# Hello1024/shared-tensor

Measured on AMD Instinct MI355X. Metric: async-DP tokens/sec GPT-2-small, higher is better.
Workload: dtype bf16; 1 GPU; model=gpt2-small, global_batch=64, seq_len=1024, parallelism=async-dp1, codec=1bit, n_params=124439808, paramsync=n/a at n_gpus=1 (no links)

## Files before the change

### build.py

```python
#!/usr/bin/env python3
import argparse
import hashlib
import os
import subprocess
import sysconfig

ROOT = os.path.dirname(os.path.abspath(__file__))
CSRC = os.path.join(ROOT, "sharedtensor_amd", "csrc")
OUT = os.path.join(ROOT, "sharedtensor_amd", "_core.so")
BUILD = os.path.join(ROOT, "build")

SOURCES = [
    "codec_cpu.cpp",
    "engine.cpp",
    "rccl_transport.cpp",
    "hip_kernels.hip",
    "ln_kernels.hip",
    "add_ln_kernels.hip",
    "add_rms_kernels.hip",
    "ce_kernels.hip",
    "gelu_kernels.hip",
    "swiglu_kernels.hip",
    "rope_kernels.hip",
    "bindings.cpp",
]

HEADERS = ["common.h", "codec_cpu.h", "engine.h", "hip_api.h", "rccl_transport.h"]


def pybind11_include():
    import pybind11
    return pybind11.get_include()


def build(force=False, debug=False, verbose=True):
    os.makedirs(BUILD, exist_ok=True)
    py_inc = sysconfig.get_paths()["include"]
    rocm = os.environ.get("ROCM_PATH", "/opt/rocm")
    hipcc = os.path.join(rocm, "bin", "hipcc")
    cxxflags = [
        "--offload-arch=gfx950",
        "-std=c++20",
        "-O3" if not debug else "-O0",
        "-g" if debug else "",
        "-fPIC",
        "-DSHAMD_WITH_HIP",
        f"-I{CSRC}",
        f"-I{py_inc}",
        f"-I{pybind11_include()}",
        f"-I{rocm}/include",
        "-Wno-unused-result",
        "-fvisibility=hidden",
        "-DNDEBUG" if not debug else "",
        "-parallel-jobs=4",
    ]
    cxxflags = [f for f in cxxflags if f]

    h = hashlib.sha256()
    for f in SOURCES + HEADERS:
        with open(os.path.join(CSRC, f), "rb") as fh:
            h.update(fh.read())
    h.update(" ".join(cxxflags).encode())
    stamp = os.path.join(BUILD, "core.stamp")
    digest = h.hexdigest()
    if not force and os.path.exists(OUT) and os.path.exists(stamp):
        with open(stamp) as fh:
            if fh.read().strip() == digest:
                if verbose:
                    print(f"[build.py] {OUT} up to date")
                return OUT

    objs = []
    procs = []
    for src in SOURCES:
        obj = os.path.join(BUILD, src.replace("/", "_") + ".o")
        objs.append(obj)
        cmd = [hipcc, "-c", os.path.join(CSRC, src), "-o", obj] + cxxflags
        if verbose:
            print("[build.py]", " ".join(cmd))
        procs.append(subprocess.Popen(cmd))
    rc = 0
    for p in procs:
        rc |= p.wait()
    if rc:
        raise RuntimeError("hipcc compilation failed")

    link = [hipcc, "-shared", "-fPIC", "-o", OUT] + objs + [
        f"-L{rocm}/lib", "-lamdhip64", "-lrccl", "-pthread",
        f"-Wl,-rpath,{rocm}/lib",
    ]
    if verbose:
        print("[build.py]", " ".join(link))
    subprocess.check_call(link)
    nm = subprocess.run(["nm", "-C", "-u", OUT], capture_output=True, text=True)
    bad = [l for l in nm.stdout.splitlines() if "shamd::" in l]
    if bad:
        raise RuntimeError("unresolved engine symbols:\n" + "\n".join(bad))
    with open(stamp, "w") as fh:
        fh.write(digest)
    if verbose:
        print(f"[build.py] built {OUT}")
    return OUT


if __name__ == "__main__":
    ap = argparse.ArgumentParser()
    ap.add_argument("--force", action="store_true")
    ap.add_argument("--debug", action="store_true")
    args = ap.parse_args()
    build(force=args.force, debug=args.debug)
```

### sharedtensor_amd/csrc/bindings.cpp

```cpp
#include <pybind11/pybind11.h>
#include <pybind11/stl.h>

#include <array>

#include "codec_cpu.h"
#include "engine.h"
#include "rccl_transport.h"

namespace py = pybind11;
using namespace shamd;

namespace {

py::tuple py_cpu_encode(int codec, uintptr_t delta, int64_t n, double scale_in,
                        uintptr_t payload_out) {
  Codec c = static_cast<Codec>(codec);
  float* d = reinterpret_cast<float*>(delta);
  float scale = scale_in < 0 ? cpu_compute_scale(c, d, n)
                             : static_cast<float>(scale_in);
  cpu_quantize(c, d, n, scale, reinterpret_cast<uint8_t*>(payload_out));
  return py::make_tuple(scale, payload_bytes(c, n));
}

void py_cpu_apply(int codec, uintptr_t payload, int64_t n, double scale,
// ... 133 lines not shown
                  reinterpret_cast<uint16_t*>(shadow_bf16),
                  static_cast<float>(lr), static_cast<float>(beta1),
                  static_cast<float>(beta2), static_cast<float>(eps),
                  static_cast<float>(wd), static_cast<float>(inv_bc1),
                  static_cast<float>(inv_bc2), n,
                  reinterpret_cast<float*>(d[0]),
                  reinterpret_cast<void*>(d[1]), reinterpret_cast<void*>(d[2]),
                  reinterpret_cast<void*>(d[3]), delta_bf16,
                  reinterpret_cast<hipStream_t>(stream));
}

void py_gpu_snapshot_capture(uintptr_t values, uintptr_t delta, uintptr_t out,
                             int64_t n, uintptr_t stream, bool delta_bf16) {
  hip_snapshot_capture(reinterpret_cast<const float*>(values),
                       reinterpret_cast<void*>(delta), delta_bf16,
                       reinterpret_cast<float*>(out), n,
                       reinterpret_cast<hipStream_t>(stream));
}

void py_gpu_add_delta_scatter(uintptr_t src, int64_t n,
                              std::vector<uintptr_t> dsts, uintptr_t stream,
                              bool delta_bf16) {
  uintptr_t d[3] = {0, 0, 0};
  for (size_t i = 0; i < dsts.size() && i < 3; ++i) d[i] = dsts[i];
  hip_add_delta_scatter(reinterpret_cast<const void*>(src), delta_bf16, n,
                        reinterpret_cast<float*>(d[0]),
                        reinterpret_cast<void*>(d[1]),
                        reinterpret_cast<void*>(d[2]),
                        reinterpret_cast<hipStream_t>(stream));
}

}

PYBIND11_MODULE(_core, m) {
  m.doc() = "MI355X-native shared-tensor engine (CDNA4 HIP + RCCL/TCP)";

  py::class_<Config>(m, "Config")
      .def(py::init<>())
      .def_readwrite("host", &Config::host)
      .def_readwrite("port", &Config::port)
      .def_readwrite("device", &Config::device)
      .def_property(
          "codec", [](const Config& c) { return static_cast<int>(c.codec); },
          [](Config& c, int v) { c.codec = static_cast<Codec>(v); })
      .def_readwrite("snapshot_join", &Config::snapshot_join)
      .def_readwrite("use_rccl", &Config::use_rccl)
      .def_readwrite("reconnect", &Config::reconnect)
      .def_readwrite("preserve_subtree", &Config::preserve_subtree)
      .def_readwrite("keepalive_s", &Config::keepalive_s)
      .def_readwrite("bw_limit", &Config::bw_limit)
      .def_readwrite("min_round_interval_s", &Config::min_round_interval_s)
      .def_readwrite("expected_children", &Config::expected_children)
      .def_readwrite("sizes", &Config::sizes)
      .def_readwrite("explicit_parent", &Config::explicit_parent)
      .def_readwrite("listen_port", &Config::listen_port)
      .def_readwrite("join_timeout_s", &Config::join_timeout_s)
      .def_readwrite("rms_sample_stride", &Config::rms_sample_stride)
      .def_readwrite("lagged_scale", &Config::lagged_scale)
      .def_readwrite("delta_bf16", &Config::delta_bf16)
      .def_readwrite("use_graphs", &Config::use_graphs);

  py::class_<Engine>(m, "Engine")
      .def(py::init<Config>())
      .def("set_values", &Engine::set_values)
      .def("set_link_buffers", &Engine::set_link_buffers)
      .def("start", &Engine::start, py::call_guard<py::gil_scoped_release>())
      .def("add_from", &Engine::add_from,
           py::call_guard<py::gil_scoped_release>())
      .def("copy_to", &Engine::copy_to,
           py::call_guard<py::gil_scoped_release>())
      .def("fused_sgd", &Engine::fused_sgd,
           py::call_guard<py::gil_scoped_release>())
      .def("fused_sgd_bf16", &Engine::fused_sgd_bf16,
           py::call_guard<py::gil_scoped_release>())
      .def("fused_adamw", &Engine::fused_adamw,
           py::call_guard<py::gil_scoped_release>())
      .def("notify_dirty", &Engine::notify_dirty)
      .def("close", &Engine::close, py::call_guard<py::gil_scoped_release>())
      .def("is_master", &Engine::is_master)
      .def("listen_port", &Engine::listen_port)
      .def("last_error", &Engine::last_error)
      .def("reconnect_count", &Engine::reconnect_count)
      .def("recent_scales_sent", &Engine::recent_scales_sent)
      .def("recent_scales_recv", &Engine::recent_scales_recv)
      .def("link_stats", [](Engine& e) {
        py::list out;
        for (auto& s : e.link_stats()) {
          py::dict d;
          d["rounds_sent"] = s.rounds_sent;
          d["rounds_recv"] = s.rounds_recv;
          d["bytes_sent"] = s.bytes_sent;
          d["bytes_recv"] = s.bytes_recv;
          d["last_scale_sent"] = s.last_scale_sent;
          d["last_scale_recv"] = s.last_scale_recv;
          d["active"] = s.active;
          d["dead"] = s.dead;
          d["peer"] = s.peer;
          d["rccl"] = s.rccl;
          out.append(d);
        }
        return out;
      });

  py::class_<DevCodec>(m, "DevCodec")
      .def(py::init<int, std::vector<int64_t>, int, bool>(), py::arg("codec"),
           py::arg("sizes"), py::arg("device"), py::arg("delta_bf16") = false)
      .def("reduce_scales", &DevCodec::reduce_scales)
      .def("quantize", &DevCodec::quantize, py::arg("delta"),
           py::arg("scales"), py::arg("payload"), py::arg("stream"),
           py::arg("stats") = 0)
      .def("finalize_scales", &DevCodec::finalize_scales)
      .def("apply", &DevCodec::apply);
  m.def("gpu_add_scatter", &py_gpu_add_scatter, py::arg("src"), py::arg("n"),
        py::arg("alpha"), py::arg("dsts"), py::arg("stream"),
        py::arg("delta_bf16") = false);
  m.def("gpu_fused_sgd", &py_gpu_fused_sgd, py::arg("mom"), py::arg("grad"),
        py::arg("lr"), py::arg("mu"), py::arg("n"), py::arg("dsts"),
        py::arg("stream"), py::arg("delta_bf16") = false);
  m.def("gpu_fused_sgd_bf16", &py_gpu_fused_sgd_bf16, py::arg("mom"),
        py::arg("grad"), py::arg("shadow"), py::arg("lr"), py::arg("mu"),
        py::arg("n"), py::arg("dsts"), py::arg("stream"),
        py::arg("delta_bf16") = false);
  m.def("gpu_fused_adamw", &py_gpu_fused_adamw, py::arg("mom"),
        py::arg("vel"), py::arg("grad"), py::arg("grad_bf16"),
        py::arg("shadow"), py::arg("lr"), py::arg("beta1"), py::arg("beta2"),
        py::arg("eps"), py::arg("wd"), py::arg("inv_bc1"), py::arg("inv_bc2"),
        py::arg("n"), py::arg("dsts"), py::arg("stream"),
        py::arg("delta_bf16") = false);
  m.def("gpu_snapshot_capture", &py_gpu_snapshot_capture, py::arg("values"),
        py::arg("delta"), py::arg("out"), py::arg("n"), py::arg("stream"),
        py::arg("delta_bf16") = false);
  m.def("gpu_add_delta_scatter", &py_gpu_add_delta_scatter, py::arg("src"),
        py::arg("n"), py::arg("dsts"), py::arg("stream"),
        py::arg("delta_bf16") = false);
  m.def("rccl_loopback_payload", &rccl_loopback_payload,
        "Self ncclSend/ncclRecv of a real payload on one device (1-rank "
        "comm): executes the non-blocking enqueue ordering + stream polling "
        "the 2-GPU xGMI links use and verifies the moved bytes.");
  m.def("rccl_self_test", &rccl_self_test,
        py::call_guard<py::gil_scoped_release>());

  m.def("gelu_fwd", [](uintptr_t x, uintptr_t y, int64_t n, uintptr_t stream) {
    hip_gelu_fwd(reinterpret_cast<const void*>(x), reinterpret_cast<void*>(y),
                 n, reinterpret_cast<hipStream_t>(stream));
  });
  m.def("gelu_bwd", [](uintptr_t dy, uintptr_t x, uintptr_t dx, int64_t n,
                       uintptr_t stream) {
    hip_gelu_bwd(reinterpret_cast<const void*>(dy),
                 reinterpret_cast<const void*>(x),
                 reinterpret_cast<void*>(dx), n,
                 reinterpret_cast<hipStream_t>(stream));
  });

  m.def("ce_fwd", [](uintptr_t logits, uintptr_t targets, uintptr_t loss,
                     uintptr_t row_m, uintptr_t row_lse, int64_t R, int64_t V,
                     uintptr_t stream) {
    hip_ce_fwd(reinterpret_cast<const void*>(logits),
               reinterpret_cast<const int32_t*>(targets),
               reinterpret_cast<float*>(loss), reinterpret_cast<float*>(row_m),
               reinterpret_cast<float*>(row_lse), R, V,
               reinterpret_cast<hipStream_t>(stream));
  });
  m.def("ce_bwd", [](uintptr_t logits, uintptr_t targets, uintptr_t row_lse,
                     uintptr_t dlogits, uintptr_t gscale_dev, double inv_r,
                     int64_t R, int64_t V, uintptr_t stream,
                     bool skip_if_unit) {
    hip_ce_bwd(reinterpret_cast<const void*>(logits),
               reinterpret_cast<const int32_t*>(targets),
               reinterpret_cast<const float*>(row_lse),
               reinterpret_cast<void*>(dlogits),
               reinterpret_cast<const float*>(gscale_dev),
               static_cast<float>(inv_r), R, V, skip_if_unit,
               reinterpret_cast<hipStream_t>(stream));
  }, py::arg("logits"), py::arg("targets"), py::arg("row_lse"),
     py::arg("dlogits"), py::arg("gscale_dev"), py::arg("inv_r"),
     py::arg("R"), py::arg("V"), py::arg("stream"),
     py::arg("skip_if_unit") = false);
  m.def("ce_fwd_grad", [](uintptr_t logits, uintptr_t targets, uintptr_t loss,
                          uintptr_t row_lse, uintptr_t dlogits, double inv_r,
                          int64_t R, int64_t V, uintptr_t stream) {
    hip_ce_fwd_grad(reinterpret_cast<const void*>(logits),
                    reinterpret_cast<const int32_t*>(targets),
                    reinterpret_cast<float*>(loss),
                    reinterpret_cast<float*>(row_lse),
                    reinterpret_cast<void*>(dlogits),
                    static_cast<float>(inv_r), R, V,
                    reinterpret_cast<hipStream_t>(stream));
  });
  m.def("ce_fwd_grad_max_v", &hip_ce_fwd_grad_max_v);

  m.def("ln_fwd", [](uintptr_t x, uintptr_t w, uintptr_t b, uintptr_t y,
                     uintptr_t mean, uintptr_t rstd, int64_t R, int C,
                     double eps, uintptr_t stream) {
    hip_ln_fwd(reinterpret_cast<const void*>(x),
               reinterpret_cast<const void*>(w),
               reinterpret_cast<const void*>(b), reinterpret_cast<void*>(y),
               reinterpret_cast<float*>(mean), reinterpret_cast<float*>(rstd),
               R, C, static_cast<float>(eps),
               reinterpret_cast<hipStream_t>(stream));
  });
  m.def("colsum_bf16", [](uintptr_t x, uintptr_t out, int64_t R, int C,
                          uintptr_t stream) {
    hip_colsum_bf16(reinterpret_cast<const void*>(x),
                    reinterpret_cast<float*>(out), R, C,
                    reinterpret_cast<hipStream_t>(stream));
  });
  m.def("swiglu_fwd", [](uintptr_t x1, uintptr_t x3, uintptr_t y, int64_t n,
                         uintptr_t stream) {
    hip_swiglu_fwd(reinterpret_cast<const void*>(x1),
                   reinterpret_cast<const void*>(x3),
                   reinterpret_cast<void*>(y), n,
                   reinterpret_cast<hipStream_t>(stream));
  });
  m.def("swiglu_bwd", [](uintptr_t dy, uintptr_t x1, uintptr_t x3,
                         uintptr_t dx1, uintptr_t dx3, int64_t n,
                         uintptr_t stream) {
    hip_swiglu_bwd(reinterpret_cast<const void*>(dy),
                   reinterpret_cast<const void*>(x1),
                   reinterpret_cast<const void*>(x3),
                   reinterpret_cast<void*>(dx1),
                   reinterpret_cast<void*>(dx3), n,
                   reinterpret_cast<hipStream_t>(stream));
  });
  m.def("rope_qk", [](uintptr_t q, uintptr_t k, uintptr_t q_out,
                      uintptr_t k_out, uintptr_t cos, uintptr_t sin,
                      int64_t B, int64_t Hq, int64_t Hkv, int64_t T,
                      int64_t D, std::array<int64_t, 3> q_strides,
                      std::array<int64_t, 3> k_strides,
                      std::array<int64_t, 3> q_out_strides,
                      std::array<int64_t, 3> k_out_strides, bool inverse,
                      uintptr_t stream) {
    auto st = [](const std::array<int64_t, 3>& a) {
      return RopeStrides{a[0], a[1], a[2]};
    };
    hip_rope_qk(reinterpret_cast<const void*>(q),
                reinterpret_cast<const void*>(k),
                reinterpret_cast<void*>(q_out),
                reinterpret_cast<void*>(k_out),
                reinterpret_cast<const float*>(cos),
                reinterpret_cast<const float*>(sin), B, Hq, Hkv, T, D,
                st(q_strides), st(k_strides), st(q_out_strides),
                st(k_out_strides), inverse,
                reinterpret_cast<hipStream_t>(stream));
  }, py::arg("q"), py::arg("k"), py::arg("q_out"), py::arg("k_out"),
     py::arg("cos"), py::arg("sin"), py::arg("B"), py::arg("Hq"),
     py::arg("Hkv"), py::arg("T"), py::arg("D"), py::arg("q_strides"),
     py::arg("k_strides"), py::arg("q_out_strides"),
     py::arg("k_out_strides"), py::arg("inverse"), py::arg("stream"));
  m.def("rms_fwd", [](uintptr_t x, uintptr_t w, uintptr_t y, uintptr_t rstd,
                      int64_t R, int C, double eps, uintptr_t stream) {
    hip_rms_fwd(reinterpret_cast<const void*>(x),
                reinterpret_cast<const void*>(w), reinterpret_cast<void*>(y),
                reinterpret_cast<float*>(rstd), R, C, static_cast<float>(eps),
                reinterpret_cast<hipStream_t>(stream));
  });
  m.def("rms_bwd", [](uintptr_t dy, uintptr_t x, uintptr_t w, uintptr_t rstd,
                      uintptr_t dx, uintptr_t dgamma, int64_t R, int C,
                      uintptr_t stream) {
    hip_rms_bwd(reinterpret_cast<const void*>(dy),
                reinterpret_cast<const void*>(x),
                reinterpret_cast<const void*>(w),
                reinterpret_cast<const float*>(rstd),
                reinterpret_cast<void*>(dx), reinterpret_cast<float*>(dgamma),
                R, C, reinterpret_cast<hipStream_t>(stream));
  });
  m.def("ln_bwd", [](uintptr_t dy, uintptr_t x, uintptr_t w, uintptr_t mean,
                     uintptr_t rstd, uintptr_t dx, uintptr_t dgamma,
                     uintptr_t dbeta, int64_t R, int C, uintptr_t stream) {
    hip_ln_bwd(reinterpret_cast<const void*>(dy),
               reinterpret_cast<const void*>(x),
               reinterpret_cast<const void*>(w),
               reinterpret_cast<const float*>(mean),
               reinterpret_cast<const float*>(rstd),
               reinterpret_cast<void*>(dx), reinterpret_cast<float*>(dgamma),
               reinterpret_cast<float*>(dbeta), R, C,
               reinterpret_cast<hipStream_t>(stream));
  });

  m.def("add_ln_supported", &hip_add_ln_supported);
  m.def("add_ln_max_blocks", &hip_add_ln_max_blocks);
  m.def("add_ln_fwd", [](uintptr_t x, uintptr_t delta, uintptr_t dbias,
                         uintptr_t w, uintptr_t b, uintptr_t x_new,
                         uintptr_t y, uintptr_t mean, uintptr_t rstd,
                         int64_t R, int C, double eps, uintptr_t stream) {
    hip_add_ln_fwd(reinterpret_cast<const void*>(x),
                   reinterpret_cast<const void*>(delta),
                   reinterpret_cast<const void*>(dbias),
                   reinterpret_cast<const void*>(w),
                   reinterpret_cast<const void*>(b),
                   reinterpret_cast<void*>(x_new), reinterpret_cast<void*>(y),
                   reinterpret_cast<float*>(mean),
                   reinterpret_cast<float*>(rstd), R, C,
                   static_cast<float>(eps),
                   reinterpret_cast<hipStream_t>(stream));
  });
  m.def("add_ln_bwd", [](uintptr_t dy, uintptr_t x_new, uintptr_t w,
                         uintptr_t mean, uintptr_t rstd, uintptr_t d_x_new,
                         uintptr_t dx_total, uintptr_t dgamma, uintptr_t dbeta,
                         uintptr_t ddbias, uintptr_t partial, int64_t R, int C,
                         uintptr_t stream) {
    hip_add_ln_bwd(reinterpret_cast<const void*>(dy),
                   reinterpret_cast<const void*>(x_new),
                   reinterpret_cast<const void*>(w),
                   reinterpret_cast<const float*>(mean),
                   reinterpret_cast<const float*>(rstd),
                   reinterpret_cast<const void*>(d_x_new),
// ... 56 lines not shown
```

### sharedtensor_amd/csrc/gelu_kernels.hip

```cpp
#include <hip/hip_runtime.h>

#include <stdexcept>
#include <string>

#include "hip_api.h"

namespace shamd {

#define HIP_CHECK_GL(expr)                                                 \
  do {                                                                     \
    hipError_t _e = (expr);                                                \
    if (_e != hipSuccess)                                                  \
      throw std::runtime_error(std::string("HIP error: ") +                \
                               hipGetErrorString(_e));                     \
  } while (0)

static __device__ __forceinline__ float gl_lo(uint32_t p) {
  return __uint_as_float(p << 16);
}
static __device__ __forceinline__ float gl_hi(uint32_t p) {
  return __uint_as_float(p & 0xFFFF0000u);
}
static __device__ __forceinline__ uint16_t gl_bf16(float f) {
  uint32_t u = __float_as_uint(f);
  if ((u & 0x7FFFFFFFu) > 0x7F800000u) return 0x7FC0;
  u += 0x7FFFu + ((u >> 16) & 1u);
  return static_cast<uint16_t>(u >> 16);
}
static __device__ __forceinline__ uint32_t gl_pack(float lo, float hi) {
  return static_cast<uint32_t>(gl_bf16(lo)) |
         (static_cast<uint32_t>(gl_bf16(hi)) << 16);
}

constexpr float GK = 0.7978845608028654f;
constexpr float GC = 0.044715f;

static __device__ __forceinline__ float gelu_f(float x) {
  float inner = GK * (x + GC * x * x * x);
  return 0.5f * x * (1.f + tanhf(inner));
}

static __device__ __forceinline__ float gelu_grad_f(float xin) {
  float x = fminf(fmaxf(xin, -10.f), 10.f);
  if (xin != xin) x = xin;
  float x2 = x * x;
  float inner = GK * x * (1.f + GC * x2);
  float t = tanhf(inner);
  float sech2 = 1.f - t * t;
  return 0.5f * (1.f + t) + 0.5f * x * sech2 * GK * (1.f + 3.f * GC * x2);
}

__global__ void k_gelu_fwd(const uint4* __restrict__ x,
                           uint4* __restrict__ y, int64_t n8) {
  int64_t g = static_cast<int64_t>(gridDim.x) * blockDim.x;
  for (int64_t i = blockIdx.x * (int64_t)blockDim.x + threadIdx.x; i < n8; i += g) {
    uint4 u = x[i];
    uint4 o;
    const uint32_t* up = &u.x;
    uint32_t* op = &o.x;
#pragma unroll
    for (int k = 0; k < 4; ++k)
      op[k] = gl_pack(gelu_f(gl_lo(up[k])), gelu_f(gl_hi(up[k])));
    y[i] = o;
  }
}

__global__ void k_gelu_bwd(const uint4* __restrict__ dy,
                           const uint4* __restrict__ x,
                           uint4* __restrict__ dx, int64_t n8) {
  int64_t g = static_cast<int64_t>(gridDim.x) * blockDim.x;
  for (int64_t i = blockIdx.x * (int64_t)blockDim.x + threadIdx.x; i < n8; i += g) {
    uint4 u = x[i], d = dy[i];
    uint4 o;
    const uint32_t* up = &u.x;
    const uint32_t* dp = &d.x;
    uint32_t* op = &o.x;
#pragma unroll
    for (int k = 0; k < 4; ++k)
      op[k] = gl_pack(gl_lo(dp[k]) * gelu_grad_f(gl_lo(up[k])),
                      gl_hi(dp[k]) * gelu_grad_f(gl_hi(up[k])));
    dx[i] = o;
  }
}

static void gelu_check_align(const void* p, const char* what) {
  if (reinterpret_cast<uintptr_t>(p) & 15u)
    throw std::runtime_error(std::string("gelu: ") + what +
                             " is not 16-byte aligned");
}

static inline int gelu_grid(int64_t npairs) {
  int64_t g = (npairs + 255) / 256;
  return static_cast<int>(g < 16384 ? (g > 0 ? g : 1) : 16384);
}

void hip_gelu_fwd(const void* x, void* y, int64_t n, hipStream_t s) {
  if (n % 8) throw std::runtime_error("gelu: n must be a multiple of 8");
  gelu_check_align(x, "x");
  gelu_check_align(y, "y");
  if (n <= 0) return;
  hipLaunchKernelGGL(k_gelu_fwd, dim3(gelu_grid(n / 8)), dim3(256), 0, s,
                     static_cast<const uint4*>(x),
                     static_cast<uint4*>(y), n / 8);
  HIP_CHECK_GL(hipGetLastError());
}

void hip_gelu_bwd(const void* dy, const void* x, void* dx, int64_t n,
                  hipStream_t s) {
  if (n % 8) throw std::runtime_error("gelu: n must be a multiple of 8");
  gelu_check_align(dy, "dy");
  gelu_check_align(x, "x");
  gelu_check_align(dx, "dx");
  if (n <= 0) return;
  hipLaunchKernelGGL(k_gelu_bwd, dim3(gelu_grid(n / 8)), dim3(256), 0, s,
                     static_cast<const uint4*>(dy),
                     static_cast<const uint4*>(x),
                     static_cast<uint4*>(dx), n / 8);
  HIP_CHECK_GL(hipGetLastError());
}

}
```

### sharedtensor_amd/csrc/hip_api.h

```cpp
#pragma once

#include <hip/hip_runtime.h>

#include "common.h"

namespace shamd {

inline int64_t align8(int64_t x) { return (x + 7) & ~int64_t(7); }

struct DevTable {
  int64_t* offs = nullptr;
  int64_t* poffs = nullptr;
  int T = 0;
  int64_t n = 0;
  int64_t pe = 0;
};


void hip_reduce_scales(Codec c, const void* delta, bool delta_bf16,
                       const DevTable& tb, void* reduce_buf, float* scales_out,
                       int sample_stride, hipStream_t s);

void hip_quantize(Codec c, void* delta, bool delta_bf16, const DevTable& tb,
                  const float* scales_dev, uint8_t* payload, hipStream_t s,
                  void* stats_out = nullptr);

void hip_finalize_scales(Codec c, const DevTable& tb, const void* reduce_buf,
                         float* scales_out, int sample_stride, hipStream_t s);

void hip_apply(Codec c, const uint8_t* payload, const DevTable& tb,
               const float* scales_dev, float* values, void* d1, void* d2,
               bool delta_bf16, hipStream_t s);

void hip_add_scatter(const float* src, int64_t n, float alpha, float* values,
                     void* d1, void* d2, void* d3, bool delta_bf16,
                     hipStream_t s);

void hip_snapshot_capture(const float* values, void* delta, bool delta_bf16,
                          float* out, int64_t n, hipStream_t s);

void hip_add_delta_scatter(const void* src_delta, bool delta_bf16, int64_t n,
                           float* values, void* d1, void* d2, hipStream_t s);

void hip_fused_sgd(float* mom, const float* grad, float lr, float momentum,
                   int64_t n, float* values, void* d1, void* d2, void* d3,
                   bool delta_bf16, hipStream_t s);

void hip_fused_sgd_bf16(float* mom, const uint16_t* grad, uint16_t* shadow,
                        float lr, float momentum, int64_t n, float* values,
                        void* d1, void* d2, void* d3, bool delta_bf16,
                        hipStream_t s);

void hip_fused_adamw(float* mom, float* vel, const void* grad, bool grad_bf16,
                     uint16_t* shadow, float lr, float beta1, float beta2,
                     float eps, float wd, float inv_bc1, float inv_bc2,
                     int64_t n, float* values, void* d1, void* d2, void* d3,
                     bool delta_bf16, hipStream_t s);

void hip_ln_fwd(const void* x, const void* w, const void* b, void* y,
                float* mean, float* rstd, int64_t R, int C, float eps,
                hipStream_t s);
void hip_ln_bwd(const void* dy, const void* x, const void* w,
                const float* mean, const float* rstd, void* dx, float* dgamma,
                float* dbeta, int64_t R, int C, hipStream_t s);

bool hip_add_ln_supported(int C);
int hip_add_ln_max_blocks();
void hip_add_ln_fwd(const void* x, const void* delta, const void* dbias,
                    const void* w, const void* b, void* x_new, void* y,
                    float* mean, float* rstd, int64_t R, int C, float eps,
                    hipStream_t s);
void hip_add_ln_bwd(const void* dy, const void* x_new, const void* w,
                    const float* mean, const float* rstd, const void* d_x_new,
                    void* dx_total, void* dgamma, void* dbeta, void* ddbias,
                    float* partial, int64_t R, int C, hipStream_t s);

void hip_colsum_bf16(const void* x, float* out, int64_t R, int C,
                     hipStream_t s);

void hip_rms_fwd(const void* x, const void* w, void* y, float* rstd,
                 int64_t R, int C, float eps, hipStream_t s);
void hip_rms_bwd(const void* dy, const void* x, const void* w,
                 const float* rstd, void* dx, float* dgamma, int64_t R, int C,
                 hipStream_t s);

bool hip_add_rms_supported(int C);
int hip_add_rms_max_blocks();
void hip_add_rms_fwd(const void* x, const void* delta, const void* w,
                     void* x_new, void* y, float* rstd, int64_t R, int C,
                     float eps, hipStream_t s);
void hip_add_rms_bwd(const void* dy, const void* x_new, const void* w,
                     const float* rstd, const void* d_x_new, void* dx_total,
                     void* dgamma, float* partial, int64_t R, int C,
                     hipStream_t s);

void hip_ce_fwd(const void* logits, const int32_t* targets, float* loss,
                float* row_m, float* row_lse, int64_t R, int64_t V,
                hipStream_t s);
void hip_ce_bwd(const void* logits, const int32_t* targets,
                const float* row_lse, void* dlogits, const float* gscale_dev,
                float inv_r, int64_t R, int64_t V, bool skip_if_unit,
                hipStream_t s);
int64_t hip_ce_fwd_grad_max_v();
void hip_ce_fwd_grad(const void* logits, const int32_t* targets, float* loss,
                     float* row_lse, void* dlogits, float inv_r, int64_t R,
                     int64_t V, hipStream_t s);

void hip_swiglu_fwd(const void* x1, const void* x3, void* y, int64_t n,
                    hipStream_t s);
void hip_swiglu_bwd(const void* dy, const void* x1, const void* x3, void* dx1,
                    void* dx3, int64_t n, hipStream_t s);

struct RopeStrides {
  int64_t b = 0, h = 0, t = 0;
};
void hip_rope_qk(const void* q, const void* k, void* q_out, void* k_out,
                 const float* cos, const float* sin, int64_t B, int64_t Hq,
                 int64_t Hkv, int64_t T, int64_t D, const RopeStrides& q_in,
                 const RopeStrides& k_in, const RopeStrides& q_os,
                 const RopeStrides& k_os, bool inverse, hipStream_t s);

void hip_gelu_fwd(const void* x, void* y, int64_t n, hipStream_t s);
void hip_gelu_bwd(const void* dy, const void* x, void* dx, int64_t n,
                  hipStream_t s);

}
```

### sharedtensor_amd/models/gpt2.py

```python
from __future__ import annotations

import math
from dataclasses import dataclass

import torch
import torch.nn as nn
import torch.nn.functional as F


@dataclass
class GPT2Config:
    vocab_size: int = 50257
    n_layer: int = 12
    n_head: int = 12
    n_embd: int = 768
    block_size: int = 1024
    dropout: float = 0.0

    @classmethod
    def small(cls):
        return cls()

    @classmethod
    def tiny(cls):
        return cls(vocab_size=256, n_layer=2, n_head=2, n_embd=64,
                   block_size=64)


FUSE_PROJ_BIAS = True


class FusedLayerNorm(nn.LayerNorm):

    def forward(self, x):
        if (x.is_cuda and x.dtype == torch.bfloat16
                and self.weight.dtype == torch.bfloat16):
            from ..ops import fused_ln
            if fused_ln.can_use(x, self.weight):
                return fused_ln.fused_layer_norm(x, self.weight, self.bias,
                                                 self.eps)
            with torch.autocast("cuda", enabled=False):
                return F.layer_norm(x, self.normalized_shape, self.weight,
                                    self.bias, self.eps)
        return super().forward(x)


def _fused_ln_ok(ln: nn.LayerNorm, x: torch.Tensor) -> bool:
    if (x.is_cuda and x.dtype == torch.bfloat16
            and ln.weight.dtype == torch.bfloat16):
        from ..ops import fused_ln
        return fused_ln.can_use(x, ln.weight)
    return False


def add_ln(ln: nn.LayerNorm, x, delta, delta_bias=None):
    if delta is None:
        return x, ln(x)
    if _fused_ln_ok(ln, x):
        from ..ops import fused_ln
        return fused_ln.fused_add_layer_norm(x, delta, ln.weight, ln.bias,
                                             ln.eps, delta_bias)
    x = x + delta
    if delta_bias is not None:
        x = x + delta_bias
    return x, ln(x)


class CausalSelfAttention(nn.Module):
    def __init__(self, cfg: GPT2Config):
        super().__init__()
        assert cfg.n_embd % cfg.n_head == 0
        self.qkv = nn.Linear(cfg.n_embd, 3 * cfg.n_embd)
        self.proj = nn.Linear(cfg.n_embd, cfg.n_embd)
        self.n_head = cfg.n_head
        self.head_dim = cfg.n_embd // cfg.n_head

    def forward(self, x, proj_bias=True):
        B, T, C = x.shape
        q, k, v = self.qkv(x).split(C, dim=2)
        q = q.view(B, T, self.n_head, self.head_dim).transpose(1, 2)
        k = k.view(B, T, self.n_head, self.head_dim).transpose(1, 2)
        v = v.view(B, T, self.n_head, self.head_dim).transpose(1, 2)
        if x.is_cuda:
            from torch.nn.attention import SDPBackend, sdpa_kernel
            with sdpa_kernel([SDPBackend.EFFICIENT_ATTENTION,
                              SDPBackend.FLASH_ATTENTION, SDPBackend.MATH],
                             set_priority=True):
                y = F.scaled_dot_product_attention(q, k, v, is_causal=True)
        else:
            y = F.scaled_dot_product_attention(q, k, v, is_causal=True)
        y = y.transpose(1, 2).contiguous().view(B, T, C)
        if not proj_bias:
            return F.linear(y, self.proj.weight)
        return self.proj(y)


class MLP(nn.Module):
    def __init__(self, cfg: GPT2Config):
        super().__init__()
        self.fc = nn.Linear(cfg.n_embd, 4 * cfg.n_embd)
        self.proj = nn.Linear(4 * cfg.n_embd, cfg.n_embd)

    def forward(self, x, proj_bias=True):
        h = F.gelu(self.fc(x), approximate="tanh")
        if not proj_bias:
            return F.linear(h, self.proj.weight)
        return self.proj(h)


class Block(nn.Module):
    def __init__(self, cfg: GPT2Config):
        super().__init__()
        self.ln1 = FusedLayerNorm(cfg.n_embd)
        self.attn = CausalSelfAttention(cfg)
        self.ln2 = FusedLayerNorm(cfg.n_embd)
        self.mlp = MLP(cfg)

    def forward(self, x, delta=None, delta_bias=None, fuse_proj_bias=False):
        x, h = add_ln(self.ln1, x, delta, delta_bias)
        fuse = fuse_proj_bias and _fused_ln_ok(self.ln2, x)
        a = self.attn(h, proj_bias=not fuse)
        x, h = add_ln(self.ln2, x, a, self.attn.proj.bias if fuse else None)
        m = self.mlp(h, proj_bias=not fuse)
        return x, m, (self.mlp.proj.bias if fuse else None)


class GPT2(nn.Module):
    def __init__(self, cfg: GPT2Config):
        super().__init__()
        self.cfg = cfg
        self.wte = nn.Embedding(cfg.vocab_size, cfg.n_embd)
        self.wpe = nn.Embedding(cfg.block_size, cfg.n_embd)
        self.blocks = nn.ModuleList(Block(cfg) for _ in range(cfg.n_layer))
        self.ln_f = FusedLayerNorm(cfg.n_embd)
        self.lm_head = nn.Linear(cfg.n_embd, cfg.vocab_size, bias=False)
        self.lm_head.weight = self.wte.weight
        self.apply(self._init)
        for name, p in self.named_parameters():
            if name.endswith("proj.weight"):
                nn.init.normal_(p, std=0.02 / math.sqrt(2 * cfg.n_layer))

    @staticmethod
    def _init(m):
        if isinstance(m, nn.Linear):
            nn.init.normal_(m.weight, std=0.02)
            if m.bias is not None:
                nn.init.zeros_(m.bias)
        elif isinstance(m, nn.Embedding):
            nn.init.normal_(m.weight, std=0.02)

    def forward(self, idx, targets=None):
        B, T = idx.shape
        pos = torch.arange(T, device=idx.device)
        x = self.wte(idx) + self.wpe(pos)
        delta = delta_bias = None
        for blk in self.blocks:
            x, delta, delta_bias = blk(x, delta, delta_bias,
                                       FUSE_PROJ_BIAS)
        _, x = add_ln(self.ln_f, x, delta, delta_bias)
        logits = self.lm_head(x)
        if targets is None:
            return logits, None
        flat = logits.view(-1, logits.size(-1))
        tgt = targets.reshape(-1)
        if flat.is_cuda and flat.dtype == torch.bfloat16:
            from ..ops import fused_ce
            if fused_ce.can_use(flat):
                return logits, fused_ce.fused_cross_entropy(flat, tgt)
        loss = F.cross_entropy(flat, tgt)
        return logits, loss

    def num_params(self) -> int:
        return sum(p.numel() for p in self.parameters())
```

Baseline: 783,500 tokens/s.

## Fuse QKV bias-grad column sum into split backward packing kernel

```diff
diff --git a/build.py b/build.py
--- a/build.py
+++ b/build.py
@@ -20,12 +20,13 @@
     "add_rms_kernels.hip",
     "ce_kernels.hip",
     "gelu_kernels.hip",
+    "bias_grad_kernels.hip",
     "swiglu_kernels.hip",
     "rope_kernels.hip",
     "bindings.cpp",
 ]
 
-HEADERS = ["common.h", "codec_cpu.h", "engine.h", "hip_api.h", "rccl_transport.h"]
+HEADERS = ["common.h", "codec_cpu.h", "engine.h", "gelu_math.h", "hip_api.h", "rccl_transport.h"]
 
 
 def pybind11_include():
diff --git a/sharedtensor_amd/csrc/bias_grad_kernels.hip b/sharedtensor_amd/csrc/bias_grad_kernels.hip
--- /dev/null
+++ b/sharedtensor_amd/csrc/bias_grad_kernels.hip
@@ -0,0 +1,242 @@
+#include <hip/hip_runtime.h>
+
+#include <stdexcept>
+#include <string>
+
+#include "gelu_math.h"
+#include "hip_api.h"
+
+namespace shamd {
+
+#define HIP_CHECK_BG(expr)                                                 \
+  do {                                                                     \
+    hipError_t _e = (expr);                                                \
+    if (_e != hipSuccess)                                                  \
+      throw std::runtime_error(std::string("HIP error: ") +                \
+                               hipGetErrorString(_e));                     \
+  } while (0)
+
+constexpr int BG_THREADS = 1024;
+constexpr int BG_TARGET_BLOCKS = 512;
+constexpr int BG_MAX_CT = 128;
+constexpr int BG_GELU_ROWS = 1;
+constexpr int BG_PACK_ROWS = 2;
+
+struct BgGeom {
+  int ct_shift;
+  int gx, gy;
+};
+
+static BgGeom bg_geom(int64_t R, int64_t n8, int rows) {
+  int shift = 0;
+  while ((2 << shift) <= BG_MAX_CT && n8 % (2 << shift) == 0) ++shift;
+  if (shift < 4) {
+    shift = 0;
+    while (shift < 4 && (1 << shift) < n8) ++shift;
+  }
+  BgGeom g;
+  g.ct_shift = shift;
+  const int ct = 1 << shift, rt = BG_THREADS >> shift;
+  const int64_t gx = (n8 + ct - 1) / ct;
+  if (gx > 65535) throw std::runtime_error("bias_grad: too many columns");
+  g.gx = static_cast<int>(gx);
+  int gymax = BG_TARGET_BLOCKS / g.gx;
+  if (gymax < 1) gymax = 1;
+  const int64_t need = (R + rows * rt - 1) / (rows * rt);
+  g.gy = static_cast<int>(need < gymax ? (need > 0 ? need : 1) : gymax);
+  return g;
+}
+
+static __device__ __forceinline__ void bg_acc(float* a, const uint4& o) {
+  const uint32_t* op = &o.x;
+#pragma unroll
+  for (int k = 0; k < 4; ++k) {
+    a[2 * k] += gl_lo(op[k]);
+    a[2 * k + 1] += gl_hi(op[k]);
+  }
+}
+
+static __device__ __forceinline__ void bg_block_partial(
+    const float* a, float* red, float* __restrict__ partial, int ct_shift,
+    int64_t N) {
+  float4* r4 = reinterpret_cast<float4*>(red);
+  r4[2 * threadIdx.x] = make_float4(a[0], a[1], a[2], a[3]);
+  r4[2 * threadIdx.x + 1] = make_float4(a[4], a[5], a[6], a[7]);
+  __syncthreads();
+  const int w = 8 << ct_shift;
+  const int rt = BG_THREADS >> ct_shift;
+  const int j = threadIdx.x;
+  const int64_t col = static_cast<int64_t>(blockIdx.x) * w + j;
+  if (j < w && col < N) {
+    float t = 0.f;
+    for (int y = 0; y < rt; ++y) t += red[y * w + j];
+    partial[static_cast<int64_t>(blockIdx.y) * N + col] = t;
+  }
+}
+
+static __device__ __forceinline__ uint4 bg_gelu_bwd8(const uint4& d,
+                                                     const uint4& u) {
+  uint4 o;
+  const uint32_t* up = &u.x;
+  const uint32_t* dp = &d.x;
+  uint32_t* op = &o.x;
+#pragma unroll
+  for (int k = 0; k < 4; ++k)
+    op[k] = gl_pack(gl_lo(dp[k]) * gelu_grad_f(gl_lo(up[k])),
+                    gl_hi(dp[k]) * gelu_grad_f(gl_hi(up[k])));
+  return o;
+}
+
+__global__ __launch_bounds__(BG_THREADS) void k_gelu_bwd_colsum(
+    const uint4* __restrict__ dy, const uint4* __restrict__ x,
+    uint4* __restrict__ dx, float* __restrict__ partial, int64_t R,
+    int64_t n8, int ct_shift) {
+  __shared__ float red[BG_THREADS * 8];
+  const int cx = threadIdx.x & ((1 << ct_shift) - 1);
+  const int ty = threadIdx.x >> ct_shift;
+  const int rt = BG_THREADS >> ct_shift;
+  const int64_t cj = (static_cast<int64_t>(blockIdx.x) << ct_shift) + cx;
+  float a[8];
+#pragma unroll
+  for (int k = 0; k < 8; ++k) a[k] = 0.f;
+  if (cj < n8) {
+    const int64_t stride = static_cast<int64_t>(gridDim.y) * rt;
+#pragma unroll 1
+    for (int64_t r = static_cast<int64_t>(blockIdx.y) * rt + ty; r < R;
+         r += stride) {
+      const int64_t i = r * n8 + cj;
+      const uint4 o = bg_gelu_bwd8(dy[i], x[i]);
+      dx[i] = o;
+      bg_acc(a, o);
+    }
+  }
+  bg_block_partial(a, red, partial, ct_shift, n8 * 8);
+}
+
+__global__ __launch_bounds__(BG_THREADS) void k_pack3_colsum(
+    const uint4* __restrict__ s0, const uint4* __restrict__ s1,
+    const uint4* __restrict__ s2, uint4* __restrict__ dst,
+    float* __restrict__ partial, int64_t R, int64_t c8, int ct_shift) {
+  __shared__ float red[BG_THREADS * 8];
+  const int cx = threadIdx.x & ((1 << ct_shift) - 1);
+  const int ty = threadIdx.x >> ct_shift;
+  const int rt = BG_THREADS >> ct_shift;
+  const int64_t n8 = 3 * c8;
+  const int64_t cj = (static_cast<int64_t>(blockIdx.x) << ct_shift) + cx;
+  float a[8];
+#pragma unroll
+  for (int k = 0; k < 8; ++k) a[k] = 0.f;
+  if (cj < n8) {
+    const int which = cj < c8 ? 0 : (cj < 2 * c8 ? 1 : 2);
+    const uint4* __restrict__ src = which == 0 ? s0 : (which == 1 ? s1 : s2);
+    const int64_t cs = cj - which * c8;
+    const int64_t stride = static_cast<int64_t>(gridDim.y) * rt;
+#pragma unroll 1
+    for (int64_t r = static_cast<int64_t>(blockIdx.y) * rt + ty; r < R;
+         r += 2 * stride) {
+      const int64_t r1 = r + stride;
+      const bool two = r1 < R;
+      const int64_t ra = two ? r1 : r;
+      const uint4 v0 = src[r * c8 + cs];
+      const uint4 v1 = src[ra * c8 + cs];
+      dst[r * n8 + cj] = v0;
+      bg_acc(a, v0);
+      if (two) {
+        dst[r1 * n8 + cj] = v1;
+        bg_acc(a, v1);
+      }
+    }
+  }
+  bg_block_partial(a, red, partial, ct_shift, n8 * 8);
+}
+
+__global__ __launch_bounds__(256) void k_bg_reduce(
+    const float* __restrict__ partial, int G, int64_t N,
+    uint16_t* __restrict__ out) {
+  __shared__ float red[8][33];
+  const int cg = threadIdx.x & 31, rg = threadIdx.x >> 5;
+  const int64_t j = static_cast<int64_t>(blockIdx.x) * 32 + cg;
+  float a = 0.f;
+  if (j < N)
+    for (int g = rg; g < G; g += 8) a += partial[static_cast<int64_t>(g) * N + j];
+  red[rg][cg] = a;
+  __syncthreads();
+  if (rg == 0 && j < N) {
+    float t = 0.f;
+#pragma unroll
+    for (int i = 0; i < 8; ++i) t += red[i][cg];
+    out[j] = gl_bf16(t);
+  }
+}
+
+static void bg_check_align(const void* p, const char* what) {
+  if (reinterpret_cast<uintptr_t>(p) & 15u)
+    throw std::runtime_error(std::string("bias_grad: ") + what +
+                             " is not 16-byte aligned");
+}
+
+static void bg_check_shape(int64_t R, int64_t N) {
+  if (R <= 0) throw std::runtime_error("bias_grad: empty input");
+  if (N <= 0 || N % 8)
+    throw std::runtime_error("bias_grad: columns must be a multiple of 8");
+}
+
+int64_t hip_bias_grad_partial_floats(int64_t N) {
+  const int64_t cap = static_cast<int64_t>(BG_TARGET_BLOCKS) * BG_MAX_CT * 8;
+  return N > cap ? N : cap;
+}
+
+int64_t hip_bias_grad_sweep_rows(int64_t R, int64_t N, bool pack) {
+  bg_check_shape(R, N);
+  const int rows = pack ? BG_PACK_ROWS : BG_GELU_ROWS;
+  const BgGeom g = bg_geom(R, N / 8, rows);
+  return rows * static_cast<int64_t>(g.gy) * (BG_THREADS >> g.ct_shift);
+}
+
+static void bg_reduce(const float* partial, int G, int64_t N, void* out,
+                      hipStream_t s) {
+  hipLaunchKernelGGL(k_bg_reduce, dim3(static_cast<uint32_t>((N + 31) / 32)),
+                     dim3(256), 0, s, partial, G, N,
+                     static_cast<uint16_t*>(out));
+  HIP_CHECK_BG(hipGetLastError());
+}
+
+void hip_gelu_bwd_colsum(const void* dy, const void* x, void* dx, void* db,
+                         float* partial, int64_t R, int64_t C,
+                         hipStream_t s) {
+  bg_check_shape(R, C);
+  bg_check_align(dy, "dy");
+  bg_check_align(x, "x");
+  bg_check_align(dx, "dx");
+  bg_check_align(partial, "partial");
+  if (!db) throw std::runtime_error("bias_grad: null db");
+  const BgGeom g = bg_geom(R, C / 8, BG_GELU_ROWS);
+  hipLaunchKernelGGL(k_gelu_bwd_colsum, dim3(g.gx, g.gy), dim3(BG_THREADS), 0,
+                     s, static_cast<const uint4*>(dy),
+                     static_cast<const uint4*>(x), static_cast<uint4*>(dx),
+                     partial, R, C / 8, g.ct_shift);
+  HIP_CHECK_BG(hipGetLastError());
+  bg_reduce(partial, g.gy, C, db, s);
+}
+
+void hip_pack3_colsum(const void* s0, const void* s1, const void* s2,
+                      void* dst, void* db, float* partial, int64_t R,
+                      int64_t C, hipStream_t s) {
+  bg_check_shape(R, C);
+  bg_check_align(s0, "src0");
+  bg_check_align(s1, "src1");
+  bg_check_align(s2, "src2");
+  bg_check_align(dst, "dst");
+  bg_check_align(partial, "partial");
+  if (!db) throw std::runtime_error("bias_grad: null db");
+  const BgGeom g = bg_geom(R, 3 * C / 8, BG_PACK_ROWS);
+  hipLaunchKernelGGL(k_pack3_colsum, dim3(g.gx, g.gy), dim3(BG_THREADS), 0, s,
+                     static_cast<const uint4*>(s0),
+                     static_cast<const uint4*>(s1),
+                     static_cast<const uint4*>(s2), static_cast<uint4*>(dst),
+                     partial, R, C / 8, g.ct_shift);
+  HIP_CHECK_BG(hipGetLastError());
+  bg_reduce(partial, g.gy, 3 * C, db, s);
+}
+
+}
diff --git a/sharedtensor_amd/csrc/bindings.cpp b/sharedtensor_amd/csrc/bindings.cpp
--- a/sharedtensor_amd/csrc/bindings.cpp
+++ b/sharedtensor_amd/csrc/bindings.cpp
@@ -309,6 +309,30 @@
                  reinterpret_cast<hipStream_t>(stream));
   });
 
+  m.def("bias_grad_partial_floats", &hip_bias_grad_partial_floats);
+  m.def("bias_grad_sweep_rows", &hip_bias_grad_sweep_rows);
+  m.def("gelu_bwd_colsum", [](uintptr_t dy, uintptr_t x, uintptr_t dx,
+                              uintptr_t db, uintptr_t partial, int64_t R,
+                              int64_t C, uintptr_t stream) {
+    hip_gelu_bwd_colsum(reinterpret_cast<const void*>(dy),
+                        reinterpret_cast<const void*>(x),
+                        reinterpret_cast<void*>(dx),
+                        reinterpret_cast<void*>(db),
+                        reinterpret_cast<float*>(partial), R, C,
+                        reinterpret_cast<hipStream_t>(stream));
+  });
+  m.def("pack3_colsum", [](uintptr_t s0, uintptr_t s1, uintptr_t s2,
+                           uintptr_t dst, uintptr_t db, uintptr_t partial,
+                           int64_t R, int64_t C, uintptr_t stream) {
+    hip_pack3_colsum(reinterpret_cast<const void*>(s0),
+                     reinterpret_cast<const void*>(s1),
+                     reinterpret_cast<const void*>(s2),
+                     reinterpret_cast<void*>(dst),
+                     reinterpret_cast<void*>(db),
+                     reinterpret_cast<float*>(partial), R, C,
+                     reinterpret_cast<hipStream_t>(stream));
+  });
+
   m.def("ce_fwd", [](uintptr_t logits, uintptr_t targets, uintptr_t loss,
                      uintptr_t row_m, uintptr_t row_lse, int64_t R, int64_t V,
                      uintptr_t stream) {
diff --git a/sharedtensor_amd/csrc/gelu_kernels.hip b/sharedtensor_amd/csrc/gelu_kernels.hip
--- a/sharedtensor_amd/csrc/gelu_kernels.hip
+++ b/sharedtensor_amd/csrc/gelu_kernels.hip
@@ -3,6 +3,7 @@
 #include <stdexcept>
 #include <string>
 
+#include "gelu_math.h"
 #include "hip_api.h"
 
 namespace shamd {
@@ -14,41 +15,6 @@
       throw std::runtime_error(std::string("HIP error: ") +                \
                                hipGetErrorString(_e));                     \
   } while (0)
-
-static __device__ __forceinline__ float gl_lo(uint32_t p) {
-  return __uint_as_float(p << 16);
-}
-static __device__ __forceinline__ float gl_hi(uint32_t p) {
-  return __uint_as_float(p & 0xFFFF0000u);
-}
-static __device__ __forceinline__ uint16_t gl_bf16(float f) {
-  uint32_t u = __float_as_uint(f);
-  if ((u & 0x7FFFFFFFu) > 0x7F800000u) return 0x7FC0;
-  u += 0x7FFFu + ((u >> 16) & 1u);
-  return static_cast<uint16_t>(u >> 16);
-}
-static __device__ __forceinline__ uint32_t gl_pack(float lo, float hi) {
-  return static_cast<uint32_t>(gl_bf16(lo)) |
-         (static_cast<uint32_t>(gl_bf16(hi)) << 16);
-}
-
-constexpr float GK = 0.7978845608028654f;
-constexpr float GC = 0.044715f;
-
-static __device__ __forceinline__ float gelu_f(float x) {
-  float inner = GK * (x + GC * x * x * x);
-  return 0.5f * x * (1.f + tanhf(inner));
-}
-
-static __device__ __forceinline__ float gelu_grad_f(float xin) {
-  float x = fminf(fmaxf(xin, -10.f), 10.f);
-  if (xin != xin) x = xin;
-  float x2 = x * x;
-  float inner = GK * x * (1.f + GC * x2);
-  float t = tanhf(inner);
-  float sech2 = 1.f - t * t;
-  return 0.5f * (1.f + t) + 0.5f * x * sech2 * GK * (1.f + 3.f * GC * x2);
-}
 
 __global__ void k_gelu_fwd(const uint4* __restrict__ x,
                            uint4* __restrict__ y, int64_t n8) {
diff --git a/sharedtensor_amd/csrc/gelu_math.h b/sharedtensor_amd/csrc/gelu_math.h
--- /dev/null
+++ b/sharedtensor_amd/csrc/gelu_math.h
@@ -0,0 +1,44 @@
+#pragma once
+
+#include <hip/hip_runtime.h>
+
+#include <cstdint>
+
+namespace shamd {
+
+static __device__ __forceinline__ float gl_lo(uint32_t p) {
+  return __uint_as_float(p << 16);
+}
+static __device__ __forceinline__ float gl_hi(uint32_t p) {
+  return __uint_as_float(p & 0xFFFF0000u);
+}
+static __device__ __forceinline__ uint16_t gl_bf16(float f) {
+  uint32_t u = __float_as_uint(f);
+  if ((u & 0x7FFFFFFFu) > 0x7F800000u) return 0x7FC0;
+  u += 0x7FFFu + ((u >> 16) & 1u);
+  return static_cast<uint16_t>(u >> 16);
+}
+static __device__ __forceinline__ uint32_t gl_pack(float lo, float hi) {
+  return static_cast<uint32_t>(gl_bf16(lo)) |
+         (static_cast<uint32_t>(gl_bf16(hi)) << 16);
+}
+
+constexpr float GK = 0.7978845608028654f;
+constexpr float GC = 0.044715f;
+
+static __device__ __forceinline__ float gelu_f(float x) {
+  float inner = GK * (x + GC * x * x * x);
+  return 0.5f * x * (1.f + tanhf(inner));
+}
+
+static __device__ __forceinline__ float gelu_grad_f(float xin) {
+  float x = fminf(fmaxf(xin, -10.f), 10.f);
+  if (xin != xin) x = xin;
+  float x2 = x * x;
+  float inner = GK * x * (1.f + GC * x2);
+  float t = tanhf(inner);
+  float sech2 = 1.f - t * t;
+  return 0.5f * (1.f + t) + 0.5f * x * sech2 * GK * (1.f + 3.f * GC * x2);
+}
+
+}
diff --git a/sharedtensor_amd/csrc/hip_api.h b/sharedtensor_amd/csrc/hip_api.h
--- a/sharedtensor_amd/csrc/hip_api.h
+++ b/sharedtensor_amd/csrc/hip_api.h
@@ -124,4 +124,12 @@
 void hip_gelu_bwd(const void* dy, const void* x, void* dx, int64_t n,
                   hipStream_t s);
 
+int64_t hip_bias_grad_partial_floats(int64_t N);
+int64_t hip_bias_grad_sweep_rows(int64_t R, int64_t N, bool pack);
+void hip_gelu_bwd_colsum(const void* dy, const void* x, void* dx, void* db,
+                         float* partial, int64_t R, int64_t C, hipStream_t s);
+void hip_pack3_colsum(const void* s0, const void* s1, const void* s2,
+                      void* dst, void* db, float* partial, int64_t R,
+                      int64_t C, hipStream_t s);
+
 }
diff --git a/sharedtensor_amd/models/gpt2.py b/sharedtensor_amd/models/gpt2.py
--- a/sharedtensor_amd/models/gpt2.py
+++ b/sharedtensor_amd/models/gpt2.py
@@ -1,6 +1,7 @@
 from __future__ import annotations
 
 import math
+import os
 from dataclasses import dataclass
 
 import torch
@@ -28,6 +29,23 @@
 
 
 FUSE_PROJ_BIAS = True
+
+FUSE_QKV_BIAS_GRAD = True
+FUSE_FC_BIAS_GRAD = False
+
+
+def _flag(env: str, default: bool) -> bool:
+    v = os.environ.get(env)
+    return default if v is None else v == "1"
+
+
+def _bias_grad_ok(flag: bool, which: str, x, lin: nn.Linear) -> bool:
+    if not (flag and x.is_cuda and x.dtype == torch.bfloat16
+            and lin.bias is not None and torch.is_grad_enabled()):
+        return False
+    from ..ops import fused_bias_grad as fb
+    check = fb.can_use_gelu if which == "gelu" else fb.can_use_qkv
+    return check(x, lin.weight, lin.bias)
 
 
 class FusedLayerNorm(nn.LayerNorm):
@@ -77,7 +95,13 @@
 
     def forward(self, x, proj_bias=True):
         B, T, C = x.shape
-        q, k, v = self.qkv(x).split(C, dim=2)
+        if _bias_grad_ok(_flag("SHTENS_FUSED_QKV_BGRAD", FUSE_QKV_BIAS_GRAD),
+                         "qkv", x, self.qkv):
+            from ..ops import fused_bias_grad
+            qkv = F.linear(x, self.qkv.weight, self.qkv.bias.detach())
+            q, k, v = fused_bias_grad.qkv_split_bgrad(qkv, self.qkv.bias)
+        else:
+            q, k, v = self.qkv(x).split(C, dim=2)
         q = q.view(B, T, self.n_head, self.head_dim).transpose(1, 2)
         k = k.view(B, T, self.n_head, self.head_dim).transpose(1, 2)
         v = v.view(B, T, self.n_head, self.head_dim).transpose(1, 2)
@@ -102,7 +126,13 @@
         self.proj = nn.Linear(4 * cfg.n_embd, cfg.n_embd)
 
     def forward(self, x, proj_bias=True):
-        h = F.gelu(self.fc(x), approximate="tanh")
+        if _bias_grad_ok(_flag("SHTENS_FUSED_GELU_BGRAD", FUSE_FC_BIAS_GRAD),
+                         "gelu", x, self.fc):
+            from ..ops import fused_bias_grad
+            pre = F.linear(x, self.fc.weight, self.fc.bias.detach())
+            h = fused_bias_grad.bias_gelu_bgrad(pre, self.fc.bias)
+        else:
+            h = F.gelu(self.fc(x), approximate="tanh")
         if not proj_bias:
             return F.linear(h, self.proj.weight)
         return self.proj(h)
diff --git a/sharedtensor_amd/ops/fused_bias_grad.py b/sharedtensor_amd/ops/fused_bias_grad.py
--- /dev/null
+++ b/sharedtensor_amd/ops/fused_bias_grad.py
@@ -0,0 +1,110 @@
+from __future__ import annotations
+
+import torch
+import torch.nn.functional as F
+
+from .. import _core
+
+_partials: dict = {}
+
+
+def _partials_for(device, ncols: int, stream: int) -> torch.Tensor:
+    key = (device.index, stream)
+    n = _core.bias_grad_partial_floats(ncols)
+    buf = _partials.get(key)
+    if buf is None or buf.numel() < n:
+        buf = torch.empty(n, dtype=torch.float32, device=device)
+        _partials[key] = buf
+    return buf
+
+
+def _bf16_cuda(*tensors) -> None:
+    for t in tensors:
+        if not t.is_cuda or t.dtype != torch.bfloat16:
+            raise TypeError("fused_bias_grad: expected a CUDA bfloat16 "
+                            f"tensor, got {t.dtype} on {t.device}")
+
+
+def _vec(t: torch.Tensor) -> torch.Tensor:
+    t = t.contiguous()
+    return t.clone() if t.data_ptr() % 16 else t
+
+
+class _BiasGeluFn(torch.autograd.Function):
+    @staticmethod
+    def forward(ctx, pre, b):
+        _bf16_cuda(pre, b)
+        if b.numel() != pre.shape[-1]:
+            raise ValueError("bias and pre-activation widths differ")
+        ctx.save_for_backward(pre)
+        return F.gelu(pre, approximate="tanh")
+
+    @staticmethod
+    def backward(ctx, dy):
+        (pre,) = ctx.saved_tensors
+        _bf16_cuda(dy)
+        C = pre.shape[-1]
+        R = pre.numel() // C
+        pre = _vec(pre)
+        dy = _vec(dy)
+        dpre = torch.empty_like(pre)
+        db = torch.empty(C, dtype=torch.bfloat16, device=pre.device)
+        if R == 0:
+            return dpre, db.zero_()
+        s = torch.cuda.current_stream(pre.device).cuda_stream
+        part = _partials_for(pre.device, C, s)
+        _core.gelu_bwd_colsum(dy.data_ptr(), pre.data_ptr(), dpre.data_ptr(),
+                              db.data_ptr(), part.data_ptr(), R, C, s)
+        return dpre, db
+
+
+class _QkvSplitFn(torch.autograd.Function):
+    @staticmethod
+    def forward(ctx, qkv, b):
+        _bf16_cuda(qkv, b)
+        if b.numel() != qkv.shape[-1] or b.numel() % 3:
+            raise ValueError("bias width must be the qkv width, 3 * C")
+        ctx.shape = qkv.shape
+        C = qkv.shape[-1] // 3
+        q, k, v = qkv.split(C, dim=-1)
+        return q, k, v
+
+    @staticmethod
+    def backward(ctx, dq, dk, dv):
+        shape = ctx.shape
+        C = shape[-1] // 3
+        _bf16_cuda(dq, dk, dv)
+        dq, dk, dv = _vec(dq), _vec(dk), _vec(dv)
+        R = dq.numel() // C
+        dqkv = torch.empty(shape, dtype=dq.dtype, device=dq.device)
+        db = torch.empty(3 * C, dtype=torch.bfloat16, device=dq.device)
+        if R == 0:
+            return dqkv, db.zero_()
+        s = torch.cuda.current_stream(dq.device).cuda_stream
+        part = _partials_for(dq.device, 3 * C, s)
+        _core.pack3_colsum(dq.data_ptr(), dk.data_ptr(), dv.data_ptr(),
+                           dqkv.data_ptr(), db.data_ptr(), part.data_ptr(),
+                           R, C, s)
+        return dqkv, db
+
+
+def bias_gelu_bgrad(pre: torch.Tensor, b: torch.Tensor) -> torch.Tensor:
+    return _BiasGeluFn.apply(pre, b)
+
+
+def qkv_split_bgrad(qkv: torch.Tensor, b: torch.Tensor):
+    return _QkvSplitFn.apply(qkv, b)
+
+
+def _common(x: torch.Tensor, w: torch.Tensor, b: torch.Tensor) -> bool:
+    return (x.is_cuda and x.dtype == torch.bfloat16
+            and w.dtype == torch.bfloat16
+            and b is not None and b.dtype == torch.bfloat16)
+
+
+def can_use_gelu(x: torch.Tensor, w: torch.Tensor, b: torch.Tensor) -> bool:
+    return _common(x, w, b) and b.numel() % 8 == 0
+
+
+def can_use_qkv(x: torch.Tensor, w: torch.Tensor, b: torch.Tensor) -> bool:
+    return _common(x, w, b) and b.numel() % 24 == 0
```

New measurement: 805,900 tokens/s (median of 6 runs). 2.9% higher.
